# epam/ai-dial-rag

Measured on AMD Instinct MI355X. Metric: retrieval_qps_10Mx384, higher is better.
Workload: dtype f32 (int8 MFMA filter with exact integer dot products and a rigorous error margin, every candidate the margin cannot exclude re-scored in f64 with the reference formula)

## Files before the change

### ai-dial-rag_amd/csrc/vec_index.hip

```cpp
#include <algorithm>
#include <cmath>
#include <cstdarg>
#include <cstdio>
#include <cstdlib>
#include <cstring>
#include <mutex>
#include <new>
#include <vector>

#include "common.h"
#include "vec_kernels.h"
#include "vec_kernels_f16.h"
#include "vec_kernels_q16.h"
#include "vec_kernels_h16.h"
#include "vec_kernels_sieve.h"
#include "vec_kernels_i8.h"
#include "vec_kernels_exact.h"

namespace mir {

static thread_local char g_err[512] = "";

void set_error(const char *fmt, ...) {
    va_list ap;
// ... 282 lines not shown
        return MIR_ERR_UNSUPPORTED;
    }
    return MIR_OK;
}


struct Carver {
    char *base;
    size_t off = 0;
    template <typename T>
    T *take(size_t count) {
        off = (off + 255) & ~(size_t)255;
        T *p = base ? reinterpret_cast<T *>(base + off) : nullptr;
        off += count * sizeof(T);
        return p;
    }
};

struct SearchBuffers {
    double *q;
    uint4 *qsplit;
    double *q_sq;
    double *q_err;
    double *q_norm;
    float *q_amax;
    float *qscale;
    uint64_t *part;
    uint64_t *gthr;
    int32_t *nflag;
    uint32_t *arrive;
    int ctl_words;
    int32_t *flagged;
    double *bound_dist;
    uint32_t *bound_row;
    uint64_t *part_exact;
    double *qt;
    uint64_t *part_sample;
    uint64_t *sv_cand;
    float *sv_candv;
    uint32_t *sv_ccount;
    SieveLists sv;
    int32_t *o_doc;
    int64_t *o_chunk;
    int64_t *o_row;
    double *o_dist;
    int32_t *o_count;
    int32_t *o_flags;
};

struct SearchPlan {
    int ngroups = 0, nwg = 1, klist = 2, qpw = 32;
    int exact_grid = 1;
    bool exact_only = false;
    int nwg_first = 0;
    uint32_t tiles_first = 0;
    bool sieve = false;
    uint32_t sample_tpw = 0;
};

static size_t carve(SearchBuffers &sb, char *base, int b, int k, int d, int ksteps, const SearchPlan &pl, bool host_api, size_t i8_rows = 0) {
    const int ngroups = pl.ngroups, nwg = pl.nwg, klist = pl.klist, qpw = pl.qpw;
    Carver c{base};
    sb.q = host_api ? c.take<double>((size_t)b * d) : nullptr;
    sb.qsplit = c.take<uint4>((size_t)ngroups * (qpw / 32) * ksteps * 128);
    sb.q_sq = c.take<double>(b);
    sb.q_err = c.take<double>(b);
    sb.q_norm = c.take<double>(b);
    sb.q_amax = c.take<float>(i8_rows ? b : 0);
    sb.qscale = c.take<float>((size_t)ngroups * std::max(128, qpw));
    sb.part = c.take<uint64_t>(pl.sieve ? 0 : (size_t)ngroups * nwg * qpw * klist);
    const size_t gthr_words = (size_t)ngroups * std::max(128, qpw), arrive_words = ((size_t)b + 1) / 2;
    const size_t count_words = pl.sieve ? (size_t)b * kSieveCountStride / 2 : 0;
    sb.ctl_words = (int)(gthr_words + 1 + 2 * arrive_words + count_words);
    sb.gthr = c.take<uint64_t>((size_t)sb.ctl_words);
    sb.nflag = base ? reinterpret_cast<int32_t *>(sb.gthr + gthr_words) : nullptr;
    sb.arrive = base ? reinterpret_cast<uint32_t *>(sb.gthr + gthr_words + 1) : nullptr;
    sb.sv.over = base ? reinterpret_cast<uint32_t *>(sb.gthr + gthr_words + 1 + arrive_words) : nullptr;
    sb.sv.count = base ? reinterpret_cast<uint32_t *>(sb.gthr + gthr_words + 1 + 2 * arrive_words) : nullptr;
    sb.flagged = c.take<int32_t>(b);
    sb.bound_dist = c.take<double>(b);
    sb.bound_row = c.take<uint32_t>(b);
    sb.part_exact = c.take<uint64_t>((size_t)b * pl.exact_grid * std::min(k, kExactRound) * 2);
    sb.qt = c.take<double>((size_t)((b + kXbQ - 1) / kXbQ) * xb_dpad(d) * kXbQ);
    sb.part_sample = c.take<uint64_t>(std::max((size_t)kSampleWgs * 128 * klist, (size_t)kSampleWgs * std::max(128, qpw)));
    const size_t sv_q = pl.sieve ? (size_t)b * kSieveQueryCap : 0;
    const size_t region = i8_rows ? (size_t)kI8Region : (size_t)kSieveRegion;
    sb.sv_cand = c.take<uint64_t>(pl.sieve ? (size_t)2 * nwg * region : 0);
    sb.sv_candv = c.take<float>(pl.sieve ? (size_t)2 * nwg * region : 0);
    sb.sv_ccount = c.take<uint32_t>(pl.sieve ? (size_t)2 * nwg * (i8_rows ? 8 : 1) : 0);
    sb.sv.rv = c.take<float>(sv_q);
    sb.sv.row = c.take<uint32_t>(sv_q);
    if (host_api) {
        sb.o_doc = c.take<int32_t>((size_t)b * k);
        sb.o_chunk = c.take<int64_t>((size_t)b * k);
        sb.o_row = c.take<int64_t>((size_t)b * k);
        sb.o_dist = c.take<double>((size_t)b * k);
        sb.o_count = c.take<int32_t>(b);
        sb.o_flags = c.take<int32_t>(b);
    } else {
        sb.o_doc = nullptr; sb.o_chunk = nullptr; sb.o_row = nullptr; sb.o_dist = nullptr;
        sb.o_count = nullptr; sb.o_flags = nullptr;
    }
    return c.off + 256;
}

static int32_t acquire_ws(mir_index *ix, hipStream_t stream, size_t need, Workspace **out) {
    Workspace *w = nullptr;
    {
        std::lock_guard<std::mutex> lk(ix->mu);
        for (size_t i = 0; i < ix->pool.size(); ++i) {
            Workspace *c = ix->pool[i];
            bool ok = !c->pending || (stream && c->last_stream == stream);
            if (!ok && hipEventQuery(c->done) == hipSuccess) {
                c->pending = false;
                ok = true;
            }
            if (ok) {
                w = c;
                ix->pool.erase(ix->pool.begin() + i);
                break;
            }
        }
    }
    if (!w) {
        w = new (std::nothrow) Workspace();
        MIR_REQUIRE(w != nullptr, "out of host memory");
        hipError_t e1 = hipStreamCreateWithFlags(&w->stream, hipStreamNonBlocking);
        hipError_t e2 = hipEventCreateWithFlags(&w->done, hipEventDisableTiming);
        if (e1 != hipSuccess || e2 != hipSuccess) {
            set_error("workspace stream/event creation failed");
            delete w;
            return MIR_ERR_HIP;
        }
    }
    if (w->cap < need) {
        if (w->pending) {
            (void)hipEventSynchronize(w->done);
            w->pending = false;
        }
        if (w->buf) (void)hipFree(w->buf);
        w->buf = nullptr;
        w->cap = 0;
        hipError_t e = hipMalloc(&w->buf, need);
        if (e != hipSuccess) {
            set_error("hipMalloc(%zu) for search workspace failed: %s", need, hipGetErrorString(e));
            std::lock_guard<std::mutex> lk(ix->mu);
            ix->pool.push_back(w);
            return MIR_ERR_HIP;
        }
        w->cap = need;
    }
    *out = w;
    return MIR_OK;
}

static void release_ws(mir_index *ix, Workspace *w, hipStream_t used, bool pending) {
    w->last_stream = used;
    w->pending = pending;
    if (pending) (void)hipEventRecord(w->done, used);
    std::lock_guard<std::mutex> lk(ix->mu);
    ix->pool.push_back(w);
}

static bool wide64_split(const mir_index *ix) { return !ix->native16 && (ix->ksteps == 32 || ix->ksteps == 48 || ix->ksteps == 64); }

template <int KIND>
static int32_t launch_scan(const mir_index *ix, const uint4 *qsplit_g, int nq, int klist, int nwg,
// ... 300 lines not shown
        prep_queries_kernel<<<dim3(prep_blocks), dim3(64), 0, stream>>>(dq, b, d, ix->ksteps, ntiles32,
                                                                                    sb.qsplit, sb.q_sq, sb.q_norm, gz, gwords);
    MIR_HIP(hipGetLastError());
    for (int g = 0; g < ngroups; ++g) {
        hipEvent_t ev0 = nullptr, ev1 = nullptr;
        auto begin_profile = [&]() -> int32_t {
            if (!ix->profiling) return MIR_OK;
            {
                std::lock_guard<std::mutex> lk(ix->mu);
                if (ix->prof_free.size() >= 2) {
                    ev0 = ix->prof_free.back(); ix->prof_free.pop_back();
                    ev1 = ix->prof_free.back(); ix->prof_free.pop_back();
                }
            }
            if (!ev0) {
                MIR_HIP(hipEventCreate(&ev0));
                MIR_HIP(hipEventCreate(&ev1));
            }
            MIR_HIP(hipEventRecord(ev0, stream));
            return MIR_OK;
        };
        const uint4 *qs = sb.qsplit + (size_t)g * (qpw / 32) * ix->ksteps * 128;
        uint64_t *pg = sb.part + (size_t)g * nwg * qpw * klist;
        const int nq = std::min(qpw, b - qpw * g);
        int32_t rc;
        if (pl.sieve) {
            uint64_t *gt = sb.gthr + (size_t)g * std::max(128, qpw);
            const int q0 = qpw * g;
            const double *qn = sb.q_norm + q0, *qsq = sb.q_sq + q0, *qerr = sb.q_err + q0;
            const int guard = metric == MIR_METRIC_EUCLIDEAN_DIST ? 1 : 0;
            const uint4 *qs16 = sb.qsplit + (size_t)g * (kQ16Queries / 16) * (ix->ksteps / 2) * 64;
            const float *qsc = sb.qscale + (size_t)g * qpw;
            auto sieve = [&](uint32_t t0, uint32_t nt, int wgs, uint64_t *cand, float *cv, uint32_t *cc, bool smp) {
                float *ps = reinterpret_cast<float *>(sb.part_sample);
                unsigned long long *st = smp ? nullptr : ix->d_stats + (t0 ? 1 : 0);
                if (use_i8) {
                    const uint32_t s0 = t0 / 2, s1 = std::min<uint32_t>((t0 + nt + 1) / 2, ix->n_stages);
                    const uint4 *qf = sb.qsplit + (size_t)g * (qpw / 16) * ix->ks64 * 64;
                    if (metric == MIR_METRIC_INNER_PRODUCT)
                        return launch_sieve_i8<SCAN_IP>(ix, qpw, sb.qscale + q0, qf, qn, qsq, qerr, nq, wgs, s0, s1 - s0, guard, gt, cand, cv, cc, ps, smp, st, stream);
                    if (metric == MIR_METRIC_COSINE_SIM)
                        return launch_sieve_i8<SCAN_COS>(ix, qpw, sb.qscale + q0, qf, qn, qsq, qerr, nq, wgs, s0, s1 - s0, guard, gt, cand, cv, cc, ps, smp, st, stream);
                    return launch_sieve_i8<SCAN_L2>(ix, qpw, sb.qscale + q0, qf, qn, qsq, qerr, nq, wgs, s0, s1 - s0, guard, gt, cand, cv, cc, ps, smp, st, stream);
                }
                if (ix->native16) {
                    if (metric == MIR_METRIC_INNER_PRODUCT) return launch_sieve16<SCAN_IP>(ix, qs16, qsc, qn, qsq, nq, wgs, t0, nt, guard, gt, cand, cv, cc, ps, smp, st, stream);
                    if (metric == MIR_METRIC_COSINE_SIM) return launch_sieve16<SCAN_COS>(ix, qs16, qsc, qn, qsq, nq, wgs, t0, nt, guard, gt, cand, cv, cc, ps, smp, st, stream);
                    return launch_sieve16<SCAN_L2>(ix, qs16, qsc, qn, qsq, nq, wgs, t0, nt, guard, gt, cand, cv, cc, ps, smp, st, stream);
                }
                if (ix->wide16) {
                    const uint4 *qw = sb.qsplit + (size_t)g * (kQ16Queries / 16) * (ix->ks16 / 2) * 128;
                    if (metric == MIR_METRIC_INNER_PRODUCT) return launch_sieve16<SCAN_IP, true>(ix, qw, nullptr, qn, qsq, nq, wgs, t0, nt, guard, gt, cand, cv, cc, ps, smp, st, stream, qerr);
                    if (metric == MIR_METRIC_COSINE_SIM) return launch_sieve16<SCAN_COS, true>(ix, qw, nullptr, qn, qsq, nq, wgs, t0, nt, guard, gt, cand, cv, cc, ps, smp, st, stream, qerr);
                    return launch_sieve16<SCAN_L2, true>(ix, qw, nullptr, qn, qsq, nq, wgs, t0, nt, guard, gt, cand, cv, cc, ps, smp, st, stream, qerr);
                }
                if (metric == MIR_METRIC_INNER_PRODUCT) return launch_sieve<SCAN_IP>(ix, qpw, qs, qn, qsq, qerr, nq, wgs, t0, nt, guard, gt, cand, cv, cc, ps, smp, st, stream);
                if (metric == MIR_METRIC_COSINE_SIM) return launch_sieve<SCAN_COS>(ix, qpw, qs, qn, qsq, qerr, nq, wgs, t0, nt, guard, gt, cand, cv, cc, ps, smp, st, stream);
                return launch_sieve<SCAN_L2>(ix, qpw, qs, qn, qsq, qerr, nq, wgs, t0, nt, guard, gt, cand, cv, cc, ps, smp, st, stream);
            };
            SieveScatterArgs ca;
            ca.q0 = q0; ca.nq = nq; ca.l = sb.sv;
            SieveSelectArgs sa;
            sa.l = sb.sv; sa.q0 = q0; sa.nq = nq; sa.k = k; sa.metric = metric; sa.d = d; sa.nan_guard = guard;
            sa.rel_err = ix->native16 ? (float)kH16RelErr : kHiHiRelErr;
            sa.extra_slop = ix->wide16 ? wide_accum_slop(ix->ks16 * 16) : 0.f;
            sa.docs = ix->d_orig; sa.docs16 = ix->d_f16; sa.doc_sq = ix->d_docsq;
            sa.dnorm = (ix->native16 || !ix->norms_spread) ? nullptr : ix->d_dnorm;
            sa.q = dq; sa.q_sq = sb.q_sq; sa.q_norm = sb.q_norm; sa.max_norm = ix->d_maxnorm;
            sa.q_err = ix->native16 ? nullptr : sb.q_err;
            sa.i8_qscale = nullptr;
            sa.i8_tparam = nullptr;
            if (use_i8) {
                sa.max_norm = ix->d_i8stats;
                sa.i8_qscale = sb.qscale;
                sa.i8_tparam = ix->d_i8tp;
                sa.dnorm = nullptr;
            }
            sa.gthr = reinterpret_cast<unsigned long long *>(gt);
            sa.chunk_ids = ix->d_chunk; sa.doc_ids = ix->d_doc; sa.row_offset = ix->row_offset;
            sa.out_doc = o_doc; sa.out_chunk = o_chunk; sa.out_row = o_row; sa.out_dist = o_dist; sa.out_count = o_count;
            sa.out_flags = o_flags; sa.nflag = sb.nflag; sa.flagged = sb.flagged; sa.stats = ix->d_stats; sa.qt = sb.qt;
            rc = sieve(0, (uint32_t)kSampleWgs * pl.sample_tpw, kSampleWgs, nullptr, nullptr, nullptr, true);
            if (rc != MIR_OK) return rc;
            sample_threshold_kernel<<<dim3(nq), dim3(256), 0, stream>>>(reinterpret_cast<const float *>(sb.part_sample), kSampleWgs, qpw,
                                                                        k, nq, reinterpret_cast<unsigned long long *>(gt));
            MIR_HIP(hipGetLastError());
            rc = begin_profile();
            if (rc != MIR_OK) return rc;
            for (int phase = pl.tiles_first ? 0 : 1; phase < 2 && rc == MIR_OK; ++phase) {
                const size_t region = use_i8 ? (size_t)kI8Region : (size_t)kSieveRegion;
                uint64_t *cand = sb.sv_cand + (size_t)phase * nwg * region;
                float *cv = sb.sv_candv + (size_t)phase * nwg * region;
                uint32_t *cc = sb.sv_ccount + (size_t)phase * nwg * (use_i8 ? 8 : 1);
                rc = phase == 0 ? sieve(0, pl.tiles_first, nwg, cand, cv, cc, false)
                                : sieve(pl.tiles_first, ix->n_tiles - pl.tiles_first, nwg, cand, cv, cc, false);
                if (rc != MIR_OK) break;
                if (phase == 1 && ev0) {
                    MIR_HIP(hipEventRecord(ev1, stream));
                    std::lock_guard<std::mutex> lk(ix->mu);
                    ix->prof_events.emplace_back(ev0, ev1);
                    ev1 = nullptr;
                }
                ca.cand = cand; ca.candv = cv; ca.ccount = cc;
                if (use_i8) sieve_scatter_i8_kernel<<<dim3(nwg * 8), dim3(256), 0, stream>>>(ca);
                else sieve_scatter_kernel<<<dim3(nwg * kSieveScatterSplit), dim3(256), 0, stream>>>(ca);
                sa.mode = phase;
                MIR_HIP(hipFuncSetAttribute(reinterpret_cast<const void *>(sieve_select_kernel), hipFuncAttributeMaxDynamicSharedMemorySize,
                                            (int)sieve_select_lds_bytes()));
                sieve_select_kernel<<<dim3(nq), dim3(kSieveSelectThreads), sieve_select_lds_bytes(), stream>>>(sa);
                MIR_HIP(hipGetLastError());
            }
            if (rc != MIR_OK) return rc;
            continue;
        }
        if (qpw != 32) {
            uint64_t *gt = sb.gthr + (size_t)g * 128;
            const float *qsc = sb.qscale + (size_t)g * qpw;
            auto run = [&](int wgs, uint32_t tiles, uint64_t *out, bool sample) {
                if (ix->layout16 || ix->native16) {
                    const double *qn = sb.q_norm + (size_t)g * qpw;
                    const uint4 *qs16 = sb.qsplit + (size_t)g * (kQ16Queries / 16) * (ix->ksteps / 2) * 64;
                    auto one = [&](int w, uint32_t t0, uint32_t nt, uint64_t *o, bool smp) {
                        if (ix->native16) {
                            if (metric == MIR_METRIC_INNER_PRODUCT) return launch_scan_h16<SCAN_IP>(ix, qs16, qsc, nq, klist, w, t0, nt, o, gt, smp, stream);
                            if (metric == MIR_METRIC_COSINE_SIM) return launch_scan_h16<SCAN_COS>(ix, qs16, qsc, nq, klist, w, t0, nt, o, gt, smp, stream);
                            return launch_scan_h16<SCAN_L2>(ix, qs16, qsc, nq, klist, w, t0, nt, o, gt, smp, stream);
                        }
                        if (metric == MIR_METRIC_INNER_PRODUCT) return launch_scan_q16<SCAN_IP>(ix, qs, qn, nq, klist, w, t0, nt, o, gt, smp, stream);
                        if (metric == MIR_METRIC_COSINE_SIM) return launch_scan_q16<SCAN_COS>(ix, qs, qn, nq, klist, w, t0, nt, o, gt, smp, stream);
                        return launch_scan_q16<SCAN_L2>(ix, qs, qn, nq, klist, w, t0, nt, o, gt, smp, stream);
                    };
                    if (sample || pl.nwg_first == 0) return one(wgs, 0, tiles, out, sample);
                    int32_t r1 = one(pl.nwg_first, 0, pl.tiles_first, out, false);
                    if (r1 != MIR_OK) return r1;
                    list_threshold_kernel<<<dim3(nq), dim3(256), 0, stream>>>(out, pl.nwg_first, qpw, klist, nq,
                                                                             reinterpret_cast<unsigned long long *>(gt));
                    return one(wgs - pl.nwg_first, pl.tiles_first, tiles - pl.tiles_first, out + (size_t)pl.nwg_first * qpw * klist, false);
                }
                if (wide64_split(ix)) {
                    if (metric == MIR_METRIC_INNER_PRODUCT) return launch_scan_f16<SCAN_IP>(ix, qs, qsc, nq, klist, wgs, tiles, out, gt, sample, stream);
                    if (metric == MIR_METRIC_COSINE_SIM) return launch_scan_f16<SCAN_COS>(ix, qs, qsc, nq, klist, wgs, tiles, out, gt, sample, stream);
                    return launch_scan_f16<SCAN_L2>(ix, qs, qsc, nq, klist, wgs, tiles, out, gt, sample, stream);
                }
                set_error("internal: no wide scan for this index");
                return (int32_t)MIR_ERR_UNSUPPORTED;
            };
            const uint32_t tpw = std::min<uint32_t>(kSampleTilesPerWg, ix->n_tiles / (4u * kSampleWgs));
            const uint32_t sample_tiles = (uint32_t)kSampleWgs * tpw;
            rc = MIR_OK;
            if (tpw >= 1) {
                rc = run(kSampleWgs, sample_tiles, sb.part_sample, true);
                if (rc == MIR_OK) {
                    sample_threshold_kernel<<<dim3(nq), dim3(256), 0, stream>>>(reinterpret_cast<const float *>(sb.part_sample),
                                                                                kSampleWgs, qpw, klist, nq,
                                                                                reinterpret_cast<unsigned long long *>(gt));
                    MIR_HIP(hipGetLastError());
                }
            }
            if (rc == MIR_OK) rc = begin_profile();
            if (rc == MIR_OK) rc = run(nwg, ix->n_tiles, pg, false);
        } else {
            rc = begin_profile();
            if (rc != MIR_OK) return rc;
            if (metric == MIR_METRIC_INNER_PRODUCT) rc = launch_scan<SCAN_IP>(ix, qs, nq, klist, nwg, pg, stream);
            else if (metric == MIR_METRIC_COSINE_SIM) rc = launch_scan<SCAN_COS>(ix, qs, nq, klist, nwg, pg, stream);
            else rc = launch_scan<SCAN_L2>(ix, qs, nq, klist, nwg, pg, stream);
        }
        if (ev1) {
// ... 682 lines not shown
```

### ai-dial-rag_amd/csrc/vec_kernels_i8.h

```cpp
#pragma once
#include "vec_kernels_sieve.h"

#ifndef I8_ABL
#define I8_ABL 0
#endif

namespace mir {

typedef int __attribute__((ext_vector_type(4))) i32x4;

constexpr int kI8StatWords = 8;
constexpr int kI8MaxK = 16;
constexpr int kI8Region = 32768;
constexpr int kI8WavePart = kI8Region / 8;
__device__ __forceinline__ void i8_margin_ab(float qn, float eq, const float *__restrict__ stats, float &A, float &B) {
    i8_margin_ab_decl(qn, eq, stats, A, B);
}
__device__ __forceinline__ float i8_margin_tile(bool l2, float A, float B, float e_t, float s_t, float sq) {
    const float m = fmaf(e_t, A, B) + 2.0f * s_t * sq;
    return l2 ? 2.0f * m : m;
}

__global__ __launch_bounds__(256) void i8_tile_scale_kernel(const float *__restrict__ src, int64_t n, int d, float4 *__restrict__ tparam) {
    __shared__ float red[4];
    const int64_t tile = blockIdx.x;
    const int64_t r0 = tile * kTileRows;
    const int64_t rows = n - r0 < kTileRows ? n - r0 : kTileRows;
    const float *p = src + r0 * (int64_t)d;
    float m = 0.f;
    for (int64_t i = threadIdx.x; i < rows * d; i += 256) m = fmaxf(m, fabsf(p[i]));
#pragma unroll
    for (int off = 32; off >= 1; off >>= 1) m = fmaxf(m, __shfl_xor(m, off, 64));
    if ((threadIdx.x & 63) == 0) red[threadIdx.x >> 6] = m;
    __syncthreads();
    if (threadIdx.x == 0) {
        m = fmaxf(fmaxf(red[0], red[1]), fmaxf(red[2], red[3]));
        const float st = m > 0.f ? m / 127.0f : 1.0f;
        tparam[tile] = make_float4(st, 0.f, 0.5f / st, 0.f);
    }
}
__global__ void i8_scale_kernel(float *__restrict__ stats, const float *__restrict__ max_norm) {
    stats[0] = max_norm[0];
    stats[7] = __builtin_inff();
}

__device__ __forceinline__ int i8_quant(float x, float inv) {
    const float r = rintf(x * inv);
    return (int)fminf(fmaxf(r, -127.0f), 127.0f);
}

__global__ __launch_bounds__(256) void pack_i8_kernel(const float *__restrict__ src, int64_t n, int d, int ks64, int64_t total_lanes,
                                                      const float4 *__restrict__ tparam, uint4 *__restrict__ dst) {
    const int64_t gid = (int64_t)blockIdx.x * 256 + threadIdx.x;
    if (gid >= total_lanes) return;
    const int lane = (int)(gid & 63);
    const int64_t blk = gid >> 6;
    const int nb = ks64 * 2;
    const int b = (int)(blk % nb);
    const int64_t tile = blk / nb;
    const int s = b >> 1, rh = b & 1;
    const int64_t row = tile * kTileRows + 16 * rh + (lane & 15);
    const int col0 = 64 * s + 16 * (lane >> 4);
    uint32_t w[4] = {0u, 0u, 0u, 0u};
    if (row < n) {
        const float inv = 1.0f / tparam[tile].x;
#pragma unroll
        for (int j = 0; j < 16; ++j) {
            const float x = col0 + j < d ? src[row * (int64_t)d + col0 + j] : 0.f;
            w[j >> 2] |= ((uint32_t)i8_quant(x, inv) & 0xffu) << (8 * (j & 3));
        }
    }
    dst[blk * 64 + lane] = make_uint4(w[0], w[1], w[2], w[3]);
}

__global__ __launch_bounds__(256) void i8_residual_kernel(const float *__restrict__ src, int64_t n, int d, const float *__restrict__ doc_sq,
                                                          float4 *__restrict__ tparam, float *__restrict__ stats) {
    const int lg = threadIdx.x & 15;
    const int64_t row = (int64_t)blockIdx.x * 16 + (threadIdx.x >> 4);
    double e2 = 0.0;
    if (row < n) {
        const float s = tparam[row / kTileRows].x;
        const float inv = 1.0f / s;
        for (int j = lg; j < d; j += 16) {
            const float x = src[row * (int64_t)d + j];
            const double r = (double)x - (double)s * (double)i8_quant(x, inv);
            e2 += r * r;
        }
    }
    e2 = group_sum<16>(e2);
    if (lg == 0 && row < n) {
        const float e = (float)sqrt(e2) * (1.0f + 1e-6f);
        atomicMax(reinterpret_cast<unsigned int *>(&tparam[row / kTileRows].y), __float_as_uint(e));
        const float a = doc_sq[row];
        const volatile float *vs = stats;
        if (e > vs[2]) atomicMax(reinterpret_cast<unsigned int *>(stats) + 2, __float_as_uint(e));
// ... 46 lines not shown
}
__global__ __launch_bounds__(64) void prep_queries_i8_quant_kernel(const double *__restrict__ q, int b, int d, int ks64, int ntiles16,
                                                                   const float *__restrict__ q_amax, uint4 *__restrict__ qfrag,
                                                                   double *__restrict__ q_err, float *__restrict__ q_scale) {
    const int lane = threadIdx.x, blk = blockIdx.x;
    if (blk < ntiles16 * ks64) {
        const int s = blk % ks64, w = blk / ks64;
        const int qi = 16 * w + (lane & 15);
        const int col0 = 64 * s + 16 * (lane >> 4);
        uint32_t wv[4] = {0u, 0u, 0u, 0u};
        const float m = qi < b ? q_amax[qi] : -1.0f;
        if (m >= 0.f) {
            const float inv = m > 0.f ? 127.0f / m : 1.0f;
#pragma unroll
            for (int j = 0; j < 16; ++j) {
                const float x = col0 + j < d ? (float)q[(int64_t)qi * d + col0 + j] : 0.f;
                wv[j >> 2] |= ((uint32_t)i8_quant(x, inv) & 0xffu) << (8 * (j & 3));
            }
        }
        qfrag[(int64_t)blk * 64 + lane] = make_uint4(wv[0], wv[1], wv[2], wv[3]);
    } else {
        const int qi = blk - ntiles16 * ks64;
        if (qi >= b) return;
        const float m = q_amax[qi];
        const bool ok = m >= 0.f;
        const float inv = m > 0.f ? 127.0f / m : 1.0f;
        const float sq = 1.0f / inv;
        double e2 = 0.0;
        for (int j = lane; j < d; j += 64) {
            const double x = q[(int64_t)qi * d + j];
            const double r = ok ? x - (double)sq * (double)i8_quant((float)x, inv) : x;
            e2 += r * r;
        }
        e2 = wave_sum(e2);
        if (lane == 0) {
            q_err[qi] = sqrt(e2);
            q_scale[qi] = sq;
        }
    }
}

__host__ __device__ constexpr int sieve_i8_stages(int nw) { return nw == 8 ? kSieveStages : 3; }
__host__ __device__ constexpr size_t sieve_i8_lds_bytes(int ks64, int nw) { return (size_t)sieve_i8_stages(nw) * (ks64 * 4 * 1024 + (64 + 8) * 4) + 64; }

template <int KS64, int KIND, bool SAMPLE, int QT, int NW>
__global__ __launch_bounds__(NW * 64, 2) void sieve_i8_kernel(const uint4 *__restrict__ docs, const float *__restrict__ aux,
                                                          const uint4 *__restrict__ qfrag, const double *__restrict__ q_norm,
                                                          const double *__restrict__ q_sq, const double *__restrict__ q_err,
                                                          const float *__restrict__ stats, const float *__restrict__ q_scale,
                                                          uint32_t n_rows, uint32_t stage0, uint32_t n_stages, int nq, int nan_guard,
                                                          const uint64_t *__restrict__ gthr, uint64_t *__restrict__ cand,
                                                          float *__restrict__ candv, uint32_t *__restrict__ ccount,
                                                          float *__restrict__ part_sample, unsigned long long *__restrict__ stat) {
    static_assert(KIND == SCAN_L2 || KIND == SCAN_IP || KIND == SCAN_COS, "scan kind");
    static_assert(QT == 1 || QT == 2 || QT == 4, "query tiles per wave");
    static_assert(NW == 8 || NW == 4, "waves per workgroup");
    constexpr int NS = sieve_i8_stages(NW);
    constexpr int APW = 64 / NW;
    constexpr int NB = KS64 * 2;
    constexpr int SB = NB * 2;
    constexpr int STAGE_U4 = SB * 64;
    constexpr int PPW = SB / NW;
    constexpr int PW = PPW + 1;
    constexpr int AS = 64 + 8;
    constexpr int D = NS - 1;
    constexpr int QPL = NW * 16 * QT;
    static_assert(SB % NW == 0, "sieve_i8: d padded to a multiple of 128");
    extern __shared__ __attribute__((aligned(16))) unsigned char smem[];
    uint4 *ring = reinterpret_cast<uint4 *>(smem);
    float *aux_lds = reinterpret_cast<float *>(smem + (size_t)NS * STAGE_U4 * 16);

    const int tid = threadIdx.x, lane = tid & 63, qc = lane & 15, jg = lane >> 4;
    const int wave8 = __builtin_amdgcn_readfirstlane(tid >> 6);
    const uint32_t G = gridDim.x;

    const float amin = KIND == SCAN_L2 ? stats[7] : 0.f;
    int qloc[QT];
    bool lane_live[QT];
    unsigned long long live_mask[QT];
    constexpr float L = KIND == SCAN_L2 ? 2.0f : 1.0f;
    const float ax_hi = KIND == SCAN_COS ? stats[6] : 1.0f;
    float tbc[QT];
    float sq[QT], mA[QT], mB[QT], P1[QT], A1[QT], guard[QT], best[QT];
    i32x4 qh[QT][KS64];
    const bool active = nq > wave8 * QT * 16;
#pragma unroll
    for (int u = 0; u < QT; ++u) {
        const int t16 = wave8 * QT + u;
        qloc[u] = t16 * 16 + qc;
        lane_live[u] = qloc[u] < nq;
        live_mask[u] = __builtin_amdgcn_ballot_w64(lane_live[u]);
        sq[u] = 1.0f; mA[u] = 0.f; mB[u] = 0.f; P1[u] = -__builtin_inff(); A1[u] = 0.f; tbc[u] = -__builtin_inff();
        guard[u] = __builtin_inff(); best[u] = -__builtin_inff();
        if (lane_live[u]) {
            const float qn = (float)q_norm[qloc[u]] * (1.0f + 1e-6f);
            const float eq = (float)q_err[qloc[u]] * (1.0f + 1e-6f);
            const bool good = qn < __builtin_inff() && eq < __builtin_inff();
            sq[u] = q_scale[qloc[u]];
            if (good) i8_margin_ab(qn, eq, stats, mA[u], mB[u]);
            if (!SAMPLE) {
                const uint64_t key = gthr[qloc[u]];
                if (key != 0 && good) {
                    const float t = key_value(key);
                    float tb = t - 2e-6f * fabsf(t);
                    tbc[u] = tb;
                    if (KIND == SCAN_COS) tb = fminf(tb * stats[4], tb * stats[5]) - 1e-6f * fabsf(tb) * stats[5];
                    P1[u] = (tb + amin - L * mB[u]) / (L * sq[u]);
                    A1[u] = mA[u] / sq[u];
                    if (!(P1[u] == P1[u]) || !(A1[u] == A1[u])) { P1[u] = -__builtin_inff(); A1[u] = 0.f; tbc[u] = -__builtin_inff(); }
                }
            } else if (nan_guard) {
                const float qs = (float)q_sq[qloc[u]];
                guard[u] = qs - 1e-5f * fabsf(qs);
            }
        }
        const uint4 *qs = qfrag + (size_t)t16 * KS64 * 64 + lane;
#pragma unroll
        for (int s = 0; s < KS64; ++s) qh[u][s] = __builtin_bit_cast(i32x4, qs[s * 64]);
    }
    const uint32_t my_stages = blockIdx.x < n_stages ? (n_stages - blockIdx.x + G - 1) / G : 0;
    const uint32_t NG = my_stages;

    auto issue = [&](uint32_t g) {
        const uint32_t stage = stage0 + blockIdx.x + g * G;
        const uint4 *src = docs + (size_t)stage * STAGE_U4 + (wave8 * PPW) * 64 + lane;
        const uint32_t dst = __builtin_amdgcn_readfirstlane(lds_addr_of(ring) + ((g % NS) * STAGE_U4 + (wave8 * PPW) * 64) * 16);
#pragma unroll
        for (int i = 0; i < PPW; ++i) glds16_b128(src + i * 64, dst + i * 1024);
        {
            const uint32_t adst = __builtin_amdgcn_readfirstlane(lds_addr_of(aux_lds) + ((g % NS) * AS + wave8 * APW) * 4);
            const float *abase = aux + (size_t)stage * AS + wave8 * APW;
            if (lane < APW + (wave8 == NW - 1 ? 8 : 0)) glds4_b32_sv(abase, (uint32_t)lane * 4u, adst);
        }
    };
#pragma unroll
    for (int u = 0; u < QT; ++u)
#pragma unroll
        for (int s = 0; s < KS64; ++s) asm volatile("" : "+v"(qh[u][s]));
    asm volatile("s_waitcnt vmcnt(0)" ::: "memory");
    for (uint32_t g = 0; g < (uint32_t)D && g < NG; ++g) issue(g);

    auto wait_stage = [&](uint32_t g) {
        const uint32_t younger = (NG - 1 - g) < (uint32_t)(D - 1) ? (NG - 1 - g) : (uint32_t)(D - 1);
        if (younger == (uint32_t)(D - 1)) asm volatile("s_waitcnt vmcnt(%0)" ::"i"((D - 1) * PW) : "memory");
        else asm volatile("s_waitcnt vmcnt(0)" ::: "memory");
    };
    uint64_t *region = cand + ((size_t)blockIdx.x * NW + wave8) * kI8WavePart;
    float *regionv = candv + ((size_t)blockIdx.x * NW + wave8) * kI8WavePart;
    const unsigned long long lt_mask = (1ull << lane) - 1ull;
    uint32_t wcount = 0;

    auto filter = [&](int u, const i32x4 &c0, const i32x4 &c1, const float (&ax)[8], uint32_t t, const float4 &tp) {
        if (SAMPLE) {
            if (lane_live[u]) {
                const float vs = L * tp.x * sq[u], mg = i8_margin_tile(KIND == SCAN_L2, mA[u], mB[u], tp.y, tp.x, sq[u]) * ax_hi;
#pragma unroll
                for (int r = 0; r < 8; ++r) {
                    const float fi = (float)(r < 4 ? c0[r & 3] : c1[r & 3]);
                    const float w = KIND == SCAN_L2 ? fmaf(vs, fi, -ax[r]) : KIND == SCAN_COS ? vs * fi * ax[r] : vs * fi;
                    if (w + mg < guard[u]) best[u] = fmaxf(best[u], w - mg);
                }
            }
            return;
        }
        const float x2 = fmaf(fmaf(-tp.y, A1[u], P1[u]), 2.0f * tp.z, -4.0f);
        const int ib = (int)__builtin_amdgcn_fmed3f(floorf(x2), -2.0e9f, 2.0e9f);
        const int m0 = max(max(c0[0], c0[1]), c0[2]), m1 = max(max(c0[3], c1[0]), c1[1]);
        const int m = max(max(max(c1[2], c1[3]), m0), m1);
        if ((__builtin_amdgcn_ballot_w64(m >= ib) & live_mask[u]) == 0ull) return;
        asm volatile("" : "+s"(t));
        const float vs = L * tp.x * sq[u];
        float bound = (fmaf(-tp.y, A1[u], P1[u]) - 2.0f * tp.x) * (L * sq[u]) - amin;
        if (KIND == SCAN_COS) bound = tbc[u] - i8_margin_tile(false, mA[u], mB[u], tp.y, tp.x, sq[u]) * ax_hi;
        const float bound_w = bound - 4e-6f * (fabsf(bound) + amin);
        float v[8];
#pragma unroll
        for (int r = 0; r < 8; ++r) {
            const float fi = (float)(r < 4 ? c0[r & 3] : c1[r & 3]);
            v[r] = KIND == SCAN_L2 ? fmaf(vs, fi, -ax[r]) : KIND == SCAN_COS ? vs * fi * ax[r] : vs * fi;
        }
        uint32_t pm = 0;
#pragma unroll
        for (int r = 0; r < 8; ++r) pm |= (uint32_t)(!(v[r] < bound_w)) << r;
        if (!lane_live[u]) pm = 0;
        if (!__any(pm != 0)) return;
        const uint32_t row0 = t * kTileRows + 4 * jg;
        if (t * kTileRows + kTileRows > n_rows) {
#pragma unroll
            for (int r = 0; r < 8; ++r)
                if (row0 + 16 * (r >> 2) + (r & 3) >= n_rows) pm &= ~(1u << r);
        }
        while (__any(pm != 0)) {
            const bool has = pm != 0;
            const int r = has ? __builtin_ctz(pm) : 0;
            const unsigned long long bal = __ballot(has);
            const uint32_t slot = wcount + (uint32_t)__popcll(bal & lt_mask);
            wcount += (uint32_t)__popcll(bal);
            float vr = v[0];
#pragma unroll
            for (int i = 1; i < 8; ++i) vr = r == i ? v[i] : vr;
            if (has && slot < (uint32_t)kI8WavePart) {
                region[slot] = ((uint64_t)(uint32_t)qloc[u] << 32) | (uint64_t)(row0 + 16 * (r >> 2) + (r & 3));
                regionv[slot] = vr;
            }
            pm &= pm - 1;
        }
    };

    i32x4 p0[QT], p1[QT];
#pragma unroll
    for (int u = 0; u < QT; ++u) { p0[u] = i32x4{0, 0, 0, 0}; p1[u] = i32x4{0, 0, 0, 0}; }
    float pax[8] = {};
    float4 ptp = make_float4(1.f, 0.f, 0.5f, 0.f);
    uint32_t pt = 0;
    bool have_prev = false;
    for (uint32_t g = 0; g < my_stages; ++g) {
        const uint32_t stage = stage0 + blockIdx.x + g * G;
#if !(I8_ABL & 4)
        wait_stage(g);
#endif
#if !(I8_ABL & 2)
        __builtin_amdgcn_s_barrier();
#endif
        if (!active) {
            if (g + D < NG) issue(g + D);
            continue;
        }
#pragma unroll
        for (int sub = 0; sub < 2; ++sub) {
            const uint4 *st = ring + (size_t)(g % NS) * STAGE_U4 + sub * (NB * 64) + lane;
            constexpr int PF = QT == 4 ? 1 : (2 < KS64 ? 2 : KS64 - 1);
            uint4 f0[PF + 1], f1[PF + 1];
#pragma unroll
            for (int i = 0; i < PF; ++i) { f0[i] = st[(2 * i + 0) * 64]; f1[i] = st[(2 * i + 1) * 64]; }
            const float4 ctp = *reinterpret_cast<const float4 *>(aux_lds + (g % NS) * AS + 64 + 4 * sub);
            float cax[8] = {};
            if (KIND != SCAN_IP) {
                const float4 a0 = *reinterpret_cast<const float4 *>(aux_lds + (g % NS) * AS + 32 * sub + 4 * jg);
                const float4 a1 = *reinterpret_cast<const float4 *>(aux_lds + (g % NS) * AS + 32 * sub + 16 + 4 * jg);
                cax[0] = a0.x; cax[1] = a0.y; cax[2] = a0.z; cax[3] = a0.w;
                cax[4] = a1.x; cax[5] = a1.y; cax[6] = a1.z; cax[7] = a1.w;
            }
            i32x4 c0[QT], c1[QT];
#pragma unroll
            for (int u = 0; u < QT; ++u) { c0[u] = i32x4{0, 0, 0, 0}; c1[u] = i32x4{0, 0, 0, 0}; }
#pragma unroll
            for (int s = 0; s < KS64; ++s) {
                if (s + PF < KS64) {
                    f0[(s + PF) % (PF + 1)] = st[(2 * (s + PF) + 0) * 64];
                    f1[(s + PF) % (PF + 1)] = st[(2 * (s + PF) + 1) * 64];
                }
                __builtin_amdgcn_sched_barrier(0);
#pragma unroll
                for (int u = 0; u < QT; ++u) {
                    c0[u] = __builtin_amdgcn_mfma_i32_16x16x64_i8(__builtin_bit_cast(i32x4, f0[s % (PF + 1)]), qh[u][s], c0[u], 0, 0, 0);
                    c1[u] = __builtin_amdgcn_mfma_i32_16x16x64_i8(__builtin_bit_cast(i32x4, f1[s % (PF + 1)]), qh[u][s], c1[u], 0, 0, 0);
                }
                if (sub == 0 && s == 0) {
                    __builtin_amdgcn_sched_barrier(0);
#if !(I8_ABL & 4)
                    if (g + D < NG) issue(g + D);
#endif
                }
#pragma unroll
                for (int u = 0; u < QT; ++u)
                    if (s == 1 + u && s < KS64 && have_prev) {
                        __builtin_amdgcn_sched_barrier(0);
#if I8_ABL & 1
                        if (g == 0xffffff)
#endif
                        filter(u, p0[u], p1[u], pax, pt, ptp);
                    }
            }
            if (KS64 < QT + 1 && have_prev) {
#pragma unroll
                for (int u = KS64 - 1; u < QT; ++u) filter(u, p0[u], p1[u], pax, pt, ptp);
            }
#pragma unroll
            for (int u = 0; u < QT; ++u) { p0[u] = c0[u]; p1[u] = c1[u]; }
#pragma unroll
            for (int i = 0; i < 8; ++i) pax[i] = cax[i];
            ptp = ctp;
            pt = stage * 2 + sub;
            have_prev = true;
        }
    }
    if (have_prev) {
#pragma unroll
        for (int u = 0; u < QT; ++u) filter(u, p0[u], p1[u], pax, pt, ptp);
    }
    if (SAMPLE) {
#pragma unroll
        for (int u = 0; u < QT; ++u) {
            const float o = __shfl_xor(best[u], 16, 64);
            const float b2 = fmaxf(best[u], o);
            if (lane_live[u] && (jg == 0 || jg == 2)) part_sample[((size_t)blockIdx.x * QPL + qloc[u]) * 2 + (jg >> 1)] = b2;
        }
        return;
    }
    if (lane == 0) {
        ccount[(size_t)blockIdx.x * NW + wave8] = wcount;
        if (stat && wcount) atomicAdd(stat, (unsigned long long)wcount);
    }
}

__global__ __launch_bounds__(256) void sieve_scatter_i8_kernel(SieveScatterArgs a) {
    __shared__ uint32_t s_cnt[256], s_base[256];
    const int tid = threadIdx.x;
    const int part = blockIdx.x;
    uint32_t cnt = a.ccount[part];
    s_cnt[tid] = 0;
    __syncthreads();
    if (cnt > (uint32_t)kI8WavePart) {
        for (int i = tid; i < a.nq; i += 256) a.l.over[a.q0 + i] = 1;
        cnt = kI8WavePart;
    }
    const uint64_t *region = a.cand + (size_t)part * kI8WavePart;
    const float *regionv = a.candv + (size_t)part * kI8WavePart;
    for (uint32_t e = tid; e < cnt; e += 256) atomicAdd(&s_cnt[(int)(region[e] >> 32) & 255], 1u);
    __syncthreads();
    {
        const uint32_t c = s_cnt[tid];
        s_base[tid] = c ? atomicAdd(&a.l.count[(size_t)(a.q0 + tid) * kSieveCountStride], c) : 0u;
        s_cnt[tid] = 0;
    }
    __syncthreads();
    for (uint32_t e = tid; e < cnt; e += 256) {
        const uint64_t key = region[e];
        const int ql = (int)(key >> 32) & 255, qi = a.q0 + ql;
        const uint32_t slot = s_base[ql] + atomicAdd(&s_cnt[ql], 1u);
        if (slot < (uint32_t)kSieveQueryCap) {
            a.l.row[(size_t)qi * kSieveQueryCap + slot] = (uint32_t)key;
            a.l.rv[(size_t)qi * kSieveQueryCap + slot] = regionv[e];
        } else {
            a.l.over[qi] = 1;
        }
    }
}

}
```

### ai-dial-rag_amd/csrc/vec_kernels_sieve.h

```cpp
#pragma once
#include "vec_kernels_q16.h"
#include "vec_kernels_h16.h"

#ifndef SIEVE_ABL
#define SIEVE_ABL 0
#endif
#ifndef SIEVE_MAX3
#define SIEVE_MAX3 1
#endif
#ifndef SIEVE_SELECT_ABL
#define SIEVE_SELECT_ABL 0
#endif
#ifndef SIEVE_PREFETCH
#define SIEVE_PREFETCH 2
#endif

namespace mir {

constexpr int kSieveStages = 6;
#ifndef MIR_SIEVE_REGION
#define MIR_SIEVE_REGION 8192
#endif
constexpr int kSieveRegion = MIR_SIEVE_REGION;
constexpr int kSieveQueryCap = 16384;
// ... 743 lines not shown
    auto to_exact_pass = [&]() {
        if (a.mode != 1) return;
        if (tid == 0) {
            atomicAdd(a.stats + 3, 1ull);
            s_slot = atomicAdd(a.nflag, 1);
            a.flagged[s_slot] = qi;
            if (a.out_flags) a.out_flags[qi] = MIR_FLAG_EXACT_PASS;
            if (a.out_count) a.out_count[qi] = 0;
        }
        __syncthreads();
        exact_publish_query(a.qt, s_slot, a.q + (size_t)qi * a.d, a.d, a.metric, a.q_norm[qi], tid, NT);
    };
    if (over) {
        to_exact_pass();
        return;
    }
    auto kth_largest = [&](const float *vals, int m) -> float {
        __syncthreads();
        if (m <= NT) sieve_wave_topk<1>(vals, m, a.k, tid, NT, part + wave * 64);
        else if (m <= 2 * NT) sieve_wave_topk<2>(vals, m, a.k, tid, NT, part + wave * 64);
        else if (m <= 4 * NT) sieve_wave_topk<4>(vals, m, a.k, tid, NT, part + wave * 64);
        else sieve_wave_topk<kSieveQueryCap / kSieveSelectThreads>(vals, m, a.k, tid, NT, part + wave * 64);
        __syncthreads();
        if (wave == 0) {
            const int nw = m <= NT ? (m + 63) / 64 : NT / 64;
            uint32_t r[16];
#pragma unroll
            for (int j = 0; j < 16; ++j) {
                const int i = j * 64 + lane;
                r[j] = i < nw * a.k ? part[(i / a.k) * 64 + i % a.k] : 0u;
            }
            uint32_t wm = 0;
            for (int t = 0; t < a.k; ++t) wm = sieve_extract_max<16>(r, lane);
            if (lane == 0) s_kv = unorderable(wm);
        }
        __syncthreads();
        return s_kv;
    };
    const float qn = (float)a.q_norm[qi] * (1.0f + 1e-6f);
    const bool l2 = !(a.metric == MIR_METRIC_INNER_PRODUCT || a.metric == MIR_METRIC_COSINE_SIM);
    const float mg = a.q_err ? hihi_margin(a.metric == MIR_METRIC_COSINE_SIM, l2, qn, (float)a.q_err[qi] * (1.0f + 1e-6f), a.max_norm) +
                                   a.extra_slop * qn * (a.metric == MIR_METRIC_COSINE_SIM ? 1.0f : a.max_norm[0]) * (l2 ? 2.0f : 1.0f)
                             : a.rel_err * qn * (a.metric == MIR_METRIC_COSINE_SIM ? 1.0f : a.max_norm[0]) * (l2 ? 2.0f : 1.0f);
    const bool i8 = a.i8_qscale != nullptr;
    const bool per_row = i8 || (a.q_err != nullptr && a.dnorm != nullptr && a.metric != MIR_METRIC_COSINE_SIM);
    const float cq = (per_row && !i8) ? hihi_coeff(l2, qn, (float)a.q_err[qi] * (1.0f + 1e-6f), a.max_norm) : 0.f;
    float i8A = 0.f, i8B = 0.f;
    const float i8sq = i8 ? a.i8_qscale[qi] : 0.f;
    if (i8) {
        const float eq = (float)a.q_err[qi] * (1.0f + 1e-6f);
        if (qn < __builtin_inff() && eq < __builtin_inff()) i8_margin_ab_decl(qn, eq, a.max_norm, i8A, i8B);
        else i8A = i8B = __builtin_inff();
    }
    auto margin_of = [&](uint32_t row) {
        if (i8) {
            const float4 tp = a.i8_tparam[row / kTileRows];
            const float m = fmaf(tp.y, i8A, i8B) + 2.0f * tp.x * i8sq;
            return l2 ? 2.0f * m : a.metric == MIR_METRIC_COSINE_SIM ? m * a.max_norm[6] : m;
        }
        return per_row ? a.dnorm[row] * cq : mg;
    };
    const float eps_m = per_row ? 0.f : 1e-6f * mg;
    float guard = __builtin_inff();
    if (a.nan_guard) {
        const float qs = (float)a.q_sq[qi];
        guard = qs - 1e-5f * fabsf(qs);
    }
    for (int e0 = 0; e0 < n; e0 += NT) {
        const int e = e0 + tid;
        bool safe = false;
        if (e < n) {
            const float v = lv[e];
            const float m = margin_of(lr[e]);
            safe = v + m < guard && v > -__builtin_inff();
            s_v[e] = safe ? v - m : -__builtin_inff();
        }
        const unsigned long long bal = __ballot(safe);
        if (bal && lane == __builtin_ctzll(bal)) atomicAdd(&s_ns, __popcll(bal));
    }
    __syncthreads();
    const int ns = s_ns;
    const bool have = ns >= a.k;
    const float kv = have ? kth_largest(s_v, n) : 0.f;
    if (a.mode == 0) {
        if (have && tid == 0) {
            const float thr = kv - 4e-6f * fabsf(kv) - eps_m;
            const unsigned long long key = (unsigned long long)orderable(thr) << 32;
            if (thr == thr && key > a.gthr[blockIdx.x]) a.gthr[blockIdx.x] = key;
        }
        if (tid == 0) atomicAdd(a.stats + 4, (unsigned long long)n);
        return;
    }
    const float cut = have ? kv - 1e-5f * fabsf(kv) - eps_m : -__builtin_inff();
    auto compact = [&](int cls, int *counter) {
        for (int e0 = 0; e0 < n; e0 += NT) {
            const int e = e0 + tid;
            bool fin = false;
            if (e < n) {
                const float lb = s_v[e];
                const bool c1 = !have || !(lb > -__builtin_inff()) || !(lb < kv);
                if (cls == 1) fin = c1;
                else if (!c1) fin = !(lb + 2.0f * margin_of(lr[e]) * (1.0f + 1e-6f) < cut);
            }
            const unsigned long long bal = __ballot(fin);
            int base = 0;
            if (bal && lane == __builtin_ctzll(bal)) base = atomicAdd(counter, __popcll(bal));
            base = __shfl(base, bal ? __builtin_ctzll(bal) : 0, 64);
            const int slot = base + __popcll(bal & ((1ull << lane) - 1ull));
            if (fin && slot < kSieveSelectCap) { s_fin[slot] = (uint16_t)e; s_row[slot] = lr[e]; }
        }
        __syncthreads();
    };
    compact(1, &s_f);
    const int f1 = s_f;
    if (tid == 0) s_f1 = f1;
    compact(2, &s_f);
    int f = s_f;
    if (f > kSieveSelectCap) {
        to_exact_pass();
        return;
    }
    const double *qv = a.q + (size_t)qi * a.d;
    const double q_sq = a.q_sq[qi], q_norm = a.q_norm[qi];
    constexpr int GW = 16, GPW = 64 / GW;
    const int sub = lane / GW, lg = lane % GW;
    const bool vec4 = (a.d & 3) == 0;
    auto evaluate = [&](int lo, int hi) {
        for (int i0 = lo + wave * GPW; i0 < hi; i0 += (NT / 64) * GPW) {
            const int i = i0 + sub;
            const bool live = i < hi;
            const uint32_t row = s_row[live ? i : i0];
            double rv, dist;
            if (vec4) {
                dist = a.docs16 ? sieve_metric_g16<_Float16>(a.docs16 + (size_t)row * a.d, qv, a.d, a.metric, a.doc_sq[row], q_sq, q_norm, lg, &rv)
                                : sieve_metric_g16<float>(a.docs + (size_t)row * a.d, qv, a.d, a.metric, a.doc_sq[row], q_sq, q_norm, lg, &rv);
            } else {
                dist = a.docs16 ? exact_metric_wave<_Float16, GW, 8>(a.docs16 + (size_t)row * a.d, qv, a.d, a.metric, a.doc_sq[row], q_sq, q_norm, lg, &rv)
                                : exact_metric_wave<float, GW, 8>(a.docs + (size_t)row * a.d, qv, a.d, a.metric, a.doc_sq[row], q_sq, q_norm, lg, &rv);
            }
            if (live && lg == 0) {
                s_d[i] = dist;
                s_x[i] = dist == dist ? (float)rv : -__builtin_inff();
            }
        }
        __syncthreads();
    };
#if SIEVE_SELECT_ABL == 1
    return;
#endif
    const bool two_rounds = f - f1 > 128;
    evaluate(0, two_rounds ? f1 : f);
#if SIEVE_SELECT_ABL == 2
    return;
#endif
    if (two_rounds) {
        for (int i0 = 0; i0 < f1; i0 += NT) {
            const int i = i0 + tid;
            const bool num = i < f1 && s_x[i] > -__builtin_inff();
            const unsigned long long bal = __ballot(num);
            if (bal && lane == __builtin_ctzll(bal)) atomicAdd(&s_nn, __popcll(bal));
        }
        __syncthreads();
        if (s_nn >= a.k) {
            const float rk = kth_largest(s_x, f1);
            const float need = rk - 4e-6f * fabsf(rk) - eps_m;
            if (tid == 0) s_f = f1;
            __syncthreads();
            for (int i0 = f1; i0 < f; i0 += NT) {
                const int i = i0 + tid;
                uint16_t e = 0;
                uint32_t er = 0;
                bool keep = false;
                if (i < f) {
                    e = s_fin[i];
                    er = s_row[i];
                    keep = !(s_v[e] + 2.0f * margin_of(er) * (1.0f + 1e-6f) < need);
                }
                __syncthreads();
                const unsigned long long bal = __ballot(keep);
                int base = 0;
                if (bal && lane == __builtin_ctzll(bal)) base = atomicAdd(&s_f, __popcll(bal));
                base = __shfl(base, bal ? __builtin_ctzll(bal) : 0, 64);
                const int slot = base + __popcll(bal & ((1ull << lane) - 1ull));
                if (keep) { s_fin[slot] = e; s_row[slot] = er; }
                __syncthreads();
            }
            f = s_f;
        }
        evaluate(f1, f);
    }
    bool pre = false;
    if (f > 256) {
        for (int i0 = 0; i0 < f; i0 += NT) {
            const int i = i0 + tid;
            if (i < f) {
                const double dd = s_d[i];
                s_x[i] = dd == dd ? -(float)dd : -__builtin_inff();
            }
        }
        if (tid == 0) s_nn = 0;
        __syncthreads();
        for (int i0 = 0; i0 < f; i0 += NT) {
            const int i = i0 + tid;
            const bool num = i < f && s_x[i] > -__builtin_inff();
            const unsigned long long bal = __ballot(num);
            if (bal && lane == __builtin_ctzll(bal)) atomicAdd(&s_nn, __popcll(bal));
        }
        __syncthreads();
        pre = s_nn >= a.k;
    }
    const float kx = pre ? kth_largest(s_x, f) : -__builtin_inff();
    const int kout = a.k < f ? a.k : f;
    for (int i = tid; i < f; i += NT) {
        if (pre && s_x[i] < kx) continue;
        const double dd = s_d[i];
        const uint32_t rr = s_row[i];
        int rank = 0;
        for (int c = 0; c < f; ++c) {
            if (pre && s_x[c] < kx) continue;
            rank += dist_before(s_d[c], s_row[c], dd, rr) ? 1 : 0;
        }
        if (rank < a.k) {
            const size_t o = (size_t)qi * a.k + rank;
            if (a.out_row) a.out_row[o] = a.row_offset + (int64_t)rr;
            if (a.out_dist) a.out_dist[o] = dd;
            if (a.out_doc) a.out_doc[o] = a.doc_ids ? a.doc_ids[rr] : 0;
            if (a.out_chunk) a.out_chunk[o] = a.chunk_ids ? a.chunk_ids[rr] : (int64_t)rr;
        }
    }
    if (tid == 0) {
        atomicAdd(a.stats + 5, (unsigned long long)f);
        atomicAdd(a.stats + 2, 1ull);
        if (a.out_count) a.out_count[qi] = kout;
        if (a.out_flags) a.out_flags[qi] = 0;
    }
}

}
```

Before: 224,600.

## Tighten sample threshold by exactly re-scoring top sampled candidates

The int8 sample pass now records, for each query, the row that achieves the best lower bound along with its value. A new threshold kernel sorts these (value,row) keys, re-scores the top-k rows exactly with the reference metric, and raises the initial global threshold to the exact k-th value when that is larger. The select path's mode 0 also evaluates the class-1 candidates exactly and tightens its threshold the same way. A higher starting threshold is meant to prune more candidates in the main sieve, which costs extra exact dot products and a bitonic sort per query.

```diff
diff --git a/ai-dial-rag_amd/csrc/vec_index.hip b/ai-dial-rag_amd/csrc/vec_index.hip
--- a/ai-dial-rag_amd/csrc/vec_index.hip
+++ b/ai-dial-rag_amd/csrc/vec_index.hip
@@ -388,7 +388,7 @@
     sb.bound_row = c.take<uint32_t>(b);
     sb.part_exact = c.take<uint64_t>((size_t)b * pl.exact_grid * std::min(k, kExactRound) * 2);
     sb.qt = c.take<double>((size_t)((b + kXbQ - 1) / kXbQ) * xb_dpad(d) * kXbQ);
-    sb.part_sample = c.take<uint64_t>(std::max((size_t)kSampleWgs * 128 * klist, (size_t)kSampleWgs * std::max(128, qpw)));
+    sb.part_sample = c.take<uint64_t>(std::max((size_t)kSampleWgs * 128 * klist, (size_t)kSampleWgs * std::max(128, qpw) * 2));
     const size_t sv_q = pl.sieve ? (size_t)b * kSieveQueryCap : 0;
     const size_t region = i8_rows ? (size_t)kI8Region : (size_t)kSieveRegion;
     sb.sv_cand = c.take<uint64_t>(pl.sieve ? (size_t)2 * nwg * region : 0);
@@ -855,8 +855,16 @@
             sa.out_flags = o_flags; sa.nflag = sb.nflag; sa.flagged = sb.flagged; sa.stats = ix->d_stats; sa.qt = sb.qt;
             rc = sieve(0, (uint32_t)kSampleWgs * pl.sample_tpw, kSampleWgs, nullptr, nullptr, nullptr, true);
             if (rc != MIR_OK) return rc;
-            sample_threshold_kernel<<<dim3(nq), dim3(256), 0, stream>>>(reinterpret_cast<const float *>(sb.part_sample), kSampleWgs, qpw,
-                                                                        k, nq, reinterpret_cast<unsigned long long *>(gt));
+            if (use_i8) {
+                SieveSampleArgs ta;
+                ta.part = reinterpret_cast<const float *>(sb.part_sample); ta.nwg = kSampleWgs; ta.qpw = qpw; ta.k = k; ta.nq = nq;
+                ta.q0 = q0; ta.d = d; ta.metric = metric; ta.docs = ix->d_orig; ta.doc_sq = ix->d_docsq;
+                ta.q = dq; ta.q_sq = sb.q_sq; ta.q_norm = sb.q_norm; ta.gthr = reinterpret_cast<unsigned long long *>(gt);
+                sieve_sample_threshold_kernel<<<dim3(nq), dim3(256), 0, stream>>>(ta);
+            } else {
+                sample_threshold_kernel<<<dim3(nq), dim3(256), 0, stream>>>(reinterpret_cast<const float *>(sb.part_sample), kSampleWgs, qpw,
+                                                                            k, nq, reinterpret_cast<unsigned long long *>(gt));
+            }
             MIR_HIP(hipGetLastError());
             rc = begin_profile();
             if (rc != MIR_OK) return rc;
diff --git a/ai-dial-rag_amd/csrc/vec_kernels_i8.h b/ai-dial-rag_amd/csrc/vec_kernels_i8.h
--- a/ai-dial-rag_amd/csrc/vec_kernels_i8.h
+++ b/ai-dial-rag_amd/csrc/vec_kernels_i8.h
@@ -11,6 +11,7 @@
 
 constexpr int kI8StatWords = 8;
 constexpr int kI8MaxK = 16;
+static_assert(kI8MaxK <= kSieveSampleMaxK, "the exact sample threshold evaluates k rows in one round");
 constexpr int kI8Region = 32768;
 constexpr int kI8WavePart = kI8Region / 8;
 __device__ __forceinline__ void i8_margin_ab(float qn, float eq, const float *__restrict__ stats, float &A, float &B) {
@@ -223,6 +224,7 @@
     const float ax_hi = KIND == SCAN_COS ? stats[6] : 1.0f;
     float tbc[QT];
     float sq[QT], mA[QT], mB[QT], P1[QT], A1[QT], guard[QT], best[QT];
+    uint32_t brow[QT];
     i32x4 qh[QT][KS64];
     const bool active = nq > wave8 * QT * 16;
 #pragma unroll
@@ -232,7 +234,7 @@
         lane_live[u] = qloc[u] < nq;
         live_mask[u] = __builtin_amdgcn_ballot_w64(lane_live[u]);
         sq[u] = 1.0f; mA[u] = 0.f; mB[u] = 0.f; P1[u] = -__builtin_inff(); A1[u] = 0.f; tbc[u] = -__builtin_inff();
-        guard[u] = __builtin_inff(); best[u] = -__builtin_inff();
+        guard[u] = __builtin_inff(); best[u] = -__builtin_inff(); brow[u] = 0;
         if (lane_live[u]) {
             const float qn = (float)q_norm[qloc[u]] * (1.0f + 1e-6f);
             const float eq = (float)q_err[qloc[u]] * (1.0f + 1e-6f);
@@ -299,7 +301,8 @@
                 for (int r = 0; r < 8; ++r) {
                     const float fi = (float)(r < 4 ? c0[r & 3] : c1[r & 3]);
                     const float w = KIND == SCAN_L2 ? fmaf(vs, fi, -ax[r]) : KIND == SCAN_COS ? vs * fi * ax[r] : vs * fi;
-                    if (w + mg < guard[u]) best[u] = fmaxf(best[u], w - mg);
+                    const uint32_t row = t * kTileRows + 4 * jg + 16 * (r >> 2) + (r & 3);
+                    if (w + mg < guard[u] && w - mg > best[u] && row < n_rows) { best[u] = w - mg; brow[u] = row; }
                 }
             }
             return;
@@ -431,11 +434,18 @@
         for (int u = 0; u < QT; ++u) filter(u, p0[u], p1[u], pax, pt, ptp);
     }
     if (SAMPLE) {
+        uint32_t *part_row = reinterpret_cast<uint32_t *>(part_sample + (size_t)gridDim.x * QPL * 2);
 #pragma unroll
         for (int u = 0; u < QT; ++u) {
             const float o = __shfl_xor(best[u], 16, 64);
-            const float b2 = fmaxf(best[u], o);
-            if (lane_live[u] && (jg == 0 || jg == 2)) part_sample[((size_t)blockIdx.x * QPL + qloc[u]) * 2 + (jg >> 1)] = b2;
+            const uint32_t orow = (uint32_t)__shfl_xor((int)brow[u], 16, 64);
+            const bool other = o > best[u];
+            const float b2 = other ? o : best[u];
+            const size_t at = ((size_t)blockIdx.x * QPL + qloc[u]) * 2 + (jg >> 1);
+            if (lane_live[u] && (jg == 0 || jg == 2)) {
+                part_sample[at] = b2;
+                part_row[at] = other ? orow : brow[u];
+            }
         }
         return;
     }
diff --git a/ai-dial-rag_amd/csrc/vec_kernels_sieve.h b/ai-dial-rag_amd/csrc/vec_kernels_sieve.h
--- a/ai-dial-rag_amd/csrc/vec_kernels_sieve.h
+++ b/ai-dial-rag_amd/csrc/vec_kernels_sieve.h
@@ -849,15 +849,6 @@
     const int ns = s_ns;
     const bool have = ns >= a.k;
     const float kv = have ? kth_largest(s_v, n) : 0.f;
-    if (a.mode == 0) {
-        if (have && tid == 0) {
-            const float thr = kv - 4e-6f * fabsf(kv) - eps_m;
-            const unsigned long long key = (unsigned long long)orderable(thr) << 32;
-            if (thr == thr && key > a.gthr[blockIdx.x]) a.gthr[blockIdx.x] = key;
-        }
-        if (tid == 0) atomicAdd(a.stats + 4, (unsigned long long)n);
-        return;
-    }
     const float cut = have ? kv - 1e-5f * fabsf(kv) - eps_m : -__builtin_inff();
     auto compact = [&](int cls, int *counter) {
         for (int e0 = 0; e0 < n; e0 += NT) {
@@ -866,7 +857,8 @@
             if (e < n) {
                 const float lb = s_v[e];
                 const bool c1 = !have || !(lb > -__builtin_inff()) || !(lb < kv);
-                if (cls == 1) fin = c1;
+                if (a.mode == 0) fin = cls == 1 && lb > -__builtin_inff() && !(lb < kv);
+                else if (cls == 1) fin = c1;
                 else if (!c1) fin = !(lb + 2.0f * margin_of(lr[e]) * (1.0f + 1e-6f) < cut);
             }
             const unsigned long long bal = __ballot(fin);
@@ -878,15 +870,6 @@
         }
         __syncthreads();
     };
-    compact(1, &s_f);
-    const int f1 = s_f;
-    if (tid == 0) s_f1 = f1;
-    compact(2, &s_f);
-    int f = s_f;
-    if (f > kSieveSelectCap) {
-        to_exact_pass();
-        return;
-    }
     const double *qv = a.q + (size_t)qi * a.d;
     const double q_sq = a.q_sq[qi], q_norm = a.q_norm[qi];
     constexpr int GW = 16, GPW = 64 / GW;
@@ -912,6 +895,46 @@
         }
         __syncthreads();
     };
+    auto count_numeric = [&](int m) {
+        for (int i0 = 0; i0 < m; i0 += NT) {
+            const int i = i0 + tid;
+            const bool num = i < m && s_x[i] > -__builtin_inff();
+            const unsigned long long bal = __ballot(num);
+            if (bal && lane == __builtin_ctzll(bal)) atomicAdd(&s_nn, __popcll(bal));
+        }
+        __syncthreads();
+    };
+    if (a.mode == 0) {
+        if (have) {
+            float thr = kv - 4e-6f * fabsf(kv) - eps_m;
+            compact(1, &s_f);
+            const int f1 = s_f;
+            if (f1 <= kSieveSelectCap) {
+                evaluate(0, f1);
+                count_numeric(f1);
+                if (s_nn >= a.k) {
+                    const float rk = kth_largest(s_x, f1);
+                    const float need = rk - 4e-6f * fabsf(rk) - eps_m;
+                    thr = need > thr ? need : thr;
+                }
+            }
+            if (tid == 0) {
+                const unsigned long long key = (unsigned long long)orderable(thr) << 32;
+                if (thr == thr && key > a.gthr[blockIdx.x]) a.gthr[blockIdx.x] = key;
+            }
+        }
+        if (tid == 0) atomicAdd(a.stats + 4, (unsigned long long)n);
+        return;
+    }
+    compact(1, &s_f);
+    const int f1 = s_f;
+    if (tid == 0) s_f1 = f1;
+    compact(2, &s_f);
+    int f = s_f;
+    if (f > kSieveSelectCap) {
+        to_exact_pass();
+        return;
+    }
 #if SIEVE_SELECT_ABL == 1
     return;
 #endif
@@ -921,13 +944,7 @@
     return;
 #endif
     if (two_rounds) {
-        for (int i0 = 0; i0 < f1; i0 += NT) {
-            const int i = i0 + tid;
-            const bool num = i < f1 && s_x[i] > -__builtin_inff();
-            const unsigned long long bal = __ballot(num);
-            if (bal && lane == __builtin_ctzll(bal)) atomicAdd(&s_nn, __popcll(bal));
-        }
-        __syncthreads();
+        count_numeric(f1);
         if (s_nn >= a.k) {
             const float rk = kth_largest(s_x, f1);
             const float need = rk - 4e-6f * fabsf(rk) - eps_m;
@@ -1003,4 +1020,73 @@
     }
 }
 
-}
+constexpr int kSieveSampleMaxK = 16;
+struct SieveSampleArgs {
+    const float *part;
+    int nwg, qpw, k, nq, q0, d, metric;
+    const float *docs, *doc_sq;
+    const double *q, *q_sq, *q_norm;
+    unsigned long long *gthr;
+};
+__global__ __launch_bounds__(256) void sieve_sample_threshold_kernel(SieveSampleArgs a) {
+    constexpr int kMaxVals = 2 * 256;
+    __shared__ unsigned long long keys[kMaxVals];
+    __shared__ float s_x[kSieveSampleMaxK];
+    const int tid = threadIdx.x, lane = tid & 63, wave = tid >> 6;
+    const int q = blockIdx.x;
+    if (q >= a.nq || a.k > kSieveSampleMaxK) return;
+    const uint32_t *prow = reinterpret_cast<const uint32_t *>(a.part + (size_t)a.nwg * a.qpw * 2);
+    const int n = 2 * a.nwg;
+    for (int e = tid; e < kMaxVals; e += 256) {
+        unsigned long long key = 0;
+        if (e < n) {
+            const size_t at = ((size_t)(e >> 1) * a.qpw + q) * 2 + (e & 1);
+            const float v = a.part[at];
+            if (v > -__builtin_inff()) key = ((unsigned long long)orderable(v) << 32) | prow[at];
+        }
+        keys[e] = key;
+    }
+    for (int size = 2; size <= kMaxVals; size <<= 1)
+        for (int stride = size >> 1; stride > 0; stride >>= 1) {
+            __syncthreads();
+            const int lo = 2 * tid - (tid & (stride - 1)), hi = lo + stride;
+            const bool desc = (lo & size) == 0;
+            const unsigned long long x = keys[lo], y = keys[hi];
+            if ((x < y) == desc) {
+                keys[lo] = y;
+                keys[hi] = x;
+            }
+        }
+    __syncthreads();
+    if (keys[a.k - 1] == 0) return;
+    const int qi = a.q0 + q;
+    const double *qv = a.q + (size_t)qi * a.d;
+    const double q_sq = a.q_sq[qi], q_norm = a.q_norm[qi];
+    const int sub = lane >> 4, lg = lane & 15;
+    for (int i0 = wave * 4; i0 < a.k; i0 += 16) {
+        const int i = i0 + sub;
+        const bool live = i < a.k;
+        const uint32_t row = (uint32_t)keys[live ? i : i0];
+        double rv, dist;
+        if ((a.d & 3) == 0)
+            dist = sieve_metric_g16<float>(a.docs + (size_t)row * a.d, qv, a.d, a.metric, a.doc_sq[row], q_sq, q_norm, lg, &rv);
+        else
+            dist = exact_metric_wave<float, 16, 8>(a.docs + (size_t)row * a.d, qv, a.d, a.metric, a.doc_sq[row], q_sq, q_norm, lg, &rv);
+        if (live && lg == 0) s_x[i] = dist == dist ? (float)rv : -__builtin_inff();
+    }
+    __syncthreads();
+    if (tid == 0) {
+        float thr = key_value(keys[a.k - 1]);
+        int nn = 0;
+        for (int i = 0; i < a.k; ++i) nn += s_x[i] > -__builtin_inff() ? 1 : 0;
+        if (nn == a.k) {
+            float rk = s_x[0];
+            for (int i = 1; i < a.k; ++i) rk = fminf(rk, s_x[i]);
+            const float need = rk - 4e-6f * fabsf(rk);
+            thr = need > thr ? need : thr;
+        }
+        a.gthr[q] = (unsigned long long)orderable(thr) << 32;
+    }
+}
+
+}
```

Measured after the change: 243,400 (median of 6 runs). 8.4% higher.
